# Ouranosinc/xclim

Hardware: AMD Instinct MI355X
Metric: grid-cells x timesteps / s (tx90p = percentile_doy + threshold_count + missing mask) (higher is better)
Workload: dtype f32; 1 GPU; tx90p (percentile_doy window 5 per 90 + threshold_count > + MissingAny) on 365x1440x720 fp32 per GPU, noleap, freq YS, time-major, resident in HBM

## Files before the change

xclim_amd/csrc/quantile.hip:

```cpp
#include <stdlib.h>

#include <type_traits>

#include "pdoy.h"

template <typename Getter>
__device__ __forceinline__ double xh_hf_quantile(int L, int n, double q, double alpha, double beta, Getter get) {
  if (L == 1) return (double)get(0);
  if (n < 2) {
    return n == 1 ? (double)get(0) : xh_nan64();
  }
  double nn = (double)n;
  double vi = nn * q + (alpha + q * (1.0 - alpha - beta)) - 1.0;
  if (vi >= nn - 1.0) return (double)get(n - 1);
  if (vi < 0.0) {
    const float v0 = get(0);
    return (v0 - v0 != 0.0f) ? (double)get(n - 1) : (double)v0;
  }
  double prev = floor(vi);
  int ip = (int)prev;
  double gamma = vi - prev;
  float left = get(ip), right = get(ip + 1);
  float diff = right - left;
  double r = (double)left + (double)diff * gamma;
// ... 47 lines not shown
      int64_t t = tb - half + k;
      okm[i] = inb && tb >= 0 && t >= 0 && t < T;
      raw[i] = xh_load<VEC>(x + (okm[i] ? t : (int64_t)0) * st + c);
    }
#pragma unroll
    for (int i = 0; i < NMAX; ++i) {
#pragma unroll
      for (int v = 0; v < VEC; ++v) {
        const uint32_t kk = okm[i] ? xh_f2key(raw[i].v[v]) : 0xFFFFFFFFu;
        key[v][i] = kk;
        nvalid[v] += (kk != 0xFFFFFFFFu) ? 1 : 0;
      }
    }
#pragma unroll
    for (int v = 0; v < VEC; ++v) {
      bitonic_regs<NMAX>(key[v]);
      auto get = [&](int idx) -> float {
        uint32_t r = 0;
#pragma unroll
        for (int i = 0; i < NMAX; ++i) r |= (i == idx) ? key[v][i] : 0u;
        return xh_key2f(r);
      };
      for (int j = 0; j < nper; ++j) {
        double r = xh_hf_quantile(N, nvalid[v], qs[j], alpha, beta, get);
        out[((int64_t)j * ndoy + d) * C + c + v] = r;
      }
    }
  }
}

__device__ __forceinline__ void ce(uint32_t& a, uint32_t& b) {
  uint32_t lo = a < b ? a : b, hi = a < b ? b : a;
  a = lo;
  b = hi;
}

template <int W>
__device__ __forceinline__ void sort_small(uint32_t (&k)[W]) {
  if (W == 1) return;
  if (W == 2) { ce(k[0], k[1 % W]); return; }
  if (W == 3) { ce(k[0], k[1 % W]); ce(k[1 % W], k[2 % W]); ce(k[0], k[1 % W]); return; }
  if (W == 5) {
    ce(k[0], k[1 % W]); ce(k[3 % W], k[4 % W]); ce(k[2 % W], k[4 % W]); ce(k[2 % W], k[3 % W]); ce(k[0], k[3 % W]);
    ce(k[0], k[2 % W]); ce(k[1 % W], k[4 % W]); ce(k[1 % W], k[3 % W]); ce(k[1 % W], k[2 % W]);
    return;
  }
#pragma unroll
  for (int r = 0; r < W; ++r) {
#pragma unroll
    for (int i = (r & 1); i + 1 < W; i += 2) ce(k[i], k[i + 1]);
  }
}

template <int W, int VEC, bool COUNT = false>
__global__ void __launch_bounds__(XH_BLOCK)
k_pdoy_slide(const float* __restrict__ x, int64_t T, int64_t C, int64_t st, int64_t t_first, int ndoy, int chunk,
             const QTab* __restrict__ qtab, int nper, double* __restrict__ out, int fast, int op = 0,
             const int32_t* __restrict__ doy_period = nullptr, int32_t* __restrict__ cnt_out = nullptr,
             int32_t* __restrict__ valid_out = nullptr) {
  __shared__ QTab s_tab[8 * (W + 1)];
  for (int i = threadIdx.x; i < nper * (W + 1); i += XH_BLOCK) s_tab[i] = qtab[i];
  __syncthreads();
  constexpr int NP = VEC == 4 ? 2 : 1;
  constexpr int GW = VEC == 4 ? 2 : 1;
  const int lane = threadIdx.x & 63;
  const int64_t wbase = ((int64_t)blockIdx.x * XH_BLOCK + (threadIdx.x & ~63)) * VEC;
  if (wbase >= C) return;
  int64_t cg[NP];
  bool okg[NP];
#pragma unroll
  for (int g = 0; g < NP; ++g) {
    cg[g] = wbase + (VEC == 4 ? 2 * lane + 128 * g : lane);
    okg[g] = cg[g] < C;
  }
  auto cell = [&](int v) -> int64_t { return cg[v / GW] + v % GW; };
  constexpr int half = W / 2;
  int d0 = blockIdx.y * chunk, d1 = d0 + chunk;
  if (d1 > ndoy) d1 = ndoy;
  uint32_t win[VEC][W];
  int n[VEC];
#pragma unroll
  for (int v = 0; v < VEC; ++v) {
    n[v] = 0;
#pragma unroll
    for (int k = 0; k < W; ++k) win[v][k] = 0xFFFFFFFFu;
  }
  auto fetch = [&](int64_t t) -> VecF<VEC> {
    const int64_t tc = t < 0 ? 0 : (t >= T ? T - 1 : t);
    const float* row = x + tc * st;
    VecF<VEC> r;
#pragma unroll
    for (int g = 0; g < NP; ++g) {
      const VecF<GW> h = xh_load<GW>(row + (okg[g] ? cg[g] : C - GW));
#pragma unroll
      for (int k = 0; k < GW; ++k) r.v[(g * GW + k) % VEC] = h.v[k];
    }
    return r;
  };
  int ccnt[VEC], cval[VEC], cper = -1;
#pragma unroll
  for (int v = 0; v < VEC; ++v) { ccnt[v] = 0; cval[v] = 0; }
  auto flush_counts = [&]() {
    if (cper >= 0) {
#pragma unroll
      for (int v = 0; v < VEC; ++v) {
        if (ccnt[v] && okg[v / GW]) atomicAdd(&cnt_out[(int64_t)cper * C + cell(v)], ccnt[v]);
        if (valid_out && cval[v] && okg[v / GW]) atomicAdd(&valid_out[(int64_t)cper * C + cell(v)], cval[v]);
        ccnt[v] = 0; cval[v] = 0;
      }
    }
  };
  auto emit = [&](int d, int j, const double (&r)[VEC], const uint32_t (&centre)[VEC]) {
    if (COUNT) {
      const int p = doy_period[d];
// ... 459 lines not shown
  hipLaunchKernelGGL(k_pdoy_lds, grid, dim3(64), lds, ctx->stream, x, T, C, st, d_tbase, nyears, ndoy, window, NP, cw, d_q, nper,
                     alpha, beta, out, d_vmap, Tv, d_doy_list, ndl);
  XH_LAUNCH_CHECK();
  return XH_OK;
}

static int launch_pdoy(xh_ctx* ctx, const float* x, int64_t T, int64_t C, int64_t st, const int32_t* d_tbase, int nyears,
                       int ndoy, int window, const double* d_q, int nper, double alpha, double beta, double* out) {
  int N = nyears * window;
  unsigned gy = (unsigned)(ndoy > 1024 ? 1024 : ndoy);
  if (N <= 8 && xh_pick_vec(x, C, st) == 4) {
    dim3 grid((unsigned)cdiv64(cdiv64(C, 4), XH_BLOCK), gy);
    hipLaunchKernelGGL((k_pdoy_reg<8, 4>), grid, dim3(XH_BLOCK), 0, ctx->stream, x, T, C, st, d_tbase, nyears, ndoy,
                       window, d_q, nper, alpha, beta, out);
  } else if (N <= 8) {
    dim3 grid((unsigned)cdiv64(C, XH_BLOCK), gy);
    hipLaunchKernelGGL((k_pdoy_reg<8, 1>), grid, dim3(XH_BLOCK), 0, ctx->stream, x, T, C, st, d_tbase, nyears, ndoy,
                       window, d_q, nper, alpha, beta, out);
  } else if (N <= 16) {
    dim3 grid((unsigned)cdiv64(C, XH_BLOCK), gy);
    hipLaunchKernelGGL((k_pdoy_reg<16, 1>), grid, dim3(XH_BLOCK), 0, ctx->stream, x, T, C, st, d_tbase, nyears, ndoy,
                       window, d_q, nper, alpha, beta, out);
  } else if (N <= 32) {
    dim3 grid((unsigned)cdiv64(C, XH_BLOCK), gy);
    hipLaunchKernelGGL((k_pdoy_reg<32, 1>), grid, dim3(XH_BLOCK), 0, ctx->stream, x, T, C, st, d_tbase, nyears, ndoy,
                       window, d_q, nper, alpha, beta, out);
  } else {
    return launch_pdoy_lds(ctx, x, T, C, st, d_tbase, nyears, ndoy, window, d_q, nper, alpha, beta, out, nullptr, T, nullptr,
                           0);
  }
  XH_LAUNCH_CHECK();
  return XH_OK;
}

static int slide_fast_mode(const QTab* tab, int nper, int W) {
  bool allmax = W > 1, allmin = W > 1;
  for (int j = 0; j < nper; ++j) {
    const QTab& e = tab[j * (W + 1) + W];
    allmax = allmax && e.lo == e.hi && e.lo == W - 1;
    allmin = allmin && e.lo == e.hi && e.lo == 0;
  }
  return allmax ? 1 : (allmin ? 2 : 0);
}

static int pdoy_impl(xh_ctx* ctx, const float* x, int64_t T, int64_t C, int64_t st, const int32_t* tbase, int nyears,
                     int ndoy, int window, const double* qh, int nper, double alpha, double beta, const int32_t* vmap,
                     int64_t Tv, double* out) {
  size_t cur = 0;
  void *d_tb = nullptr, *d_q = nullptr, *d_vmap = nullptr;
  const int N = nyears * window;
  bool contiguous = !vmap && nyears == 1 && nper <= 8 && (window == 3 || window == 5 || window == 7) && tbase[0] >= 0;
  for (int d = 1; contiguous && d < ndoy; ++d) contiguous = tbase[d] == tbase[0] + d;
  if (contiguous) {
    QTab tab[8 * 8];
    build_qtab(window, qh, nper, alpha, beta, tab);
    void* d_tab = nullptr;
    int rc = xh_scratch_upload(ctx, &cur, tab, sizeof(QTab) * (size_t)nper * (window + 1), &d_tab);
    if (rc) return rc;
    int chunk = 32;
    if (const char* e = xh_diag_env("XH_PDOY_SLIDE_CHUNK")) chunk = atoi(e) > 0 ? atoi(e) : chunk;
    const int vec = slide_vec(x, C, st, out);
    dim3 grid((unsigned)cdiv64(cdiv64(C, vec), XH_BLOCK), (unsigned)((ndoy + chunk - 1) / chunk));
#define XH_SLIDE(W, V)                                                                                              \
  hipLaunchKernelGGL((k_pdoy_slide<W, V>), grid, dim3(XH_BLOCK), 0, ctx->stream, x, T, C, st, (int64_t)tbase[0], ndoy, \
                     chunk, (const QTab*)d_tab, nper, out, slide_fast_mode(tab, nper, window))
    if (vec == 4) {
      if (window == 3) XH_SLIDE(3, 4); else if (window == 5) XH_SLIDE(5, 4); else XH_SLIDE(7, 4);
    } else {
      if (window == 3) XH_SLIDE(3, 1); else if (window == 5) XH_SLIDE(5, 1); else XH_SLIDE(7, 1);
    }
#undef XH_SLIDE
    XH_LAUNCH_CHECK();
    return XH_OK;
  }
  int rc = xh_scratch_upload(ctx, &cur, tbase, sizeof(int32_t) * (size_t)nyears * ndoy, &d_tb);
  if (rc) return rc;
  rc = xh_scratch_upload(ctx, &cur, qh, sizeof(double) * nper, &d_q);
  if (rc) return rc;
  if (vmap) {
    rc = xh_scratch_upload(ctx, &cur, vmap, sizeof(int32_t) * (size_t)Tv, &d_vmap);
    if (rc) return rc;
  }
  if (!vmap && N <= 32)
    return launch_pdoy(ctx, x, T, C, st, (const int32_t*)d_tb, nyears, ndoy, window, (const double*)d_q, nper, alpha, beta,
                       out);
  const bool mergeable = N > 32 && nyears <= 64 && (window == 3 || window == 5 || window == 7) && nper <= 16;
  if (!mergeable)
    return launch_pdoy_lds(ctx, x, T, C, st, (const int32_t*)d_tb, nyears, ndoy, window, (const double*)d_q, nper, alpha,
                           beta, out, (const int32_t*)d_vmap, Tv, nullptr, 0);
  uint8_t* regular = (uint8_t*)malloc((size_t)ndoy);
  int32_t* irregular = (int32_t*)malloc(sizeof(int32_t) * (size_t)ndoy);
  QTab* tab = (QTab*)malloc(sizeof(QTab) * (size_t)nper * (N + 1));
  if (!regular || !irregular || !tab) {
    free(regular); free(irregular); free(tab);
    xh_set_error("xh_percentile_doy: out of host memory");
    return XH_ERR_ARG;
  }
  const int nirr = pdoy_regular_flags(tbase, nyears, ndoy, window, T, vmap, Tv, regular, irregular);
  build_qtab(N, qh, nper, alpha, beta, tab);
  int32_t jtop[64], jbot[64], jrest[64];
  int ntop = 0, nbot = 0, nrest = 0;
  for (int j = 0; j < nper; ++j) {
    int dt = 0, db = 0;
    for (int n = 0; n <= N; ++n) {
      const QTab& e = tab[j * (N + 1) + n];
      if (e.lo < 0) continue;
      if (n - e.lo > dt) dt = n - e.lo;
      if (e.hi + 1 > db) db = e.hi + 1;
    }
    if (dt <= 16) jtop[ntop++] = j;
    else if (db <= 16) jbot[nbot++] = j;
    else jrest[nrest++] = j;
  }
  auto ring_depth = [&](const int32_t* js, int nj, int* pKT, int* pKB) {
    int kt = 1, kb = 0;
    for (int jj = 0; jj < nj; ++jj)
      for (int n = 0; n <= N; ++n) {
        const QTab& e = tab[js[jj] * (N + 1) + n];
// ... 36 lines not shown
  if (nbot) {
    rc = xh_launch_pdoy_top16(ctx, x, T, C, st, (const int32_t*)d_tb, nyears, ndoy, window, (const QTab*)d_tab,
                              (const int32_t*)d_jbot, nbot, 1, out, (const int32_t*)d_vmap, Tv, (const uint8_t*)d_reg);
    if (rc) return rc;
  }
  if (nrest == 0 && nirr == 0) return XH_OK;
  if (nrest) {
    const int rw = xh_launch_pdoy_walk(ctx, x, T, C, st, (const int32_t*)d_tb, nyears, ndoy, window, (const QTab*)d_tab,
                                       (const int32_t*)d_jrest, nrest, out, (const int32_t*)d_vmap, Tv, (const uint8_t*)d_reg);
    if (rw == XH_OK) nrest = 0;
    else if (rw != XH_ERR_NOTIMPL) return rw;
    if (nrest == 0 && nirr == 0) return XH_OK;
  }
  const size_t lds = ((size_t)window * (KT + KB) * 64 + (size_t)window * 64) * sizeof(uint32_t);
  const size_t lds_a = ((size_t)window * (KTa + KBa) * 64 + (size_t)window * 64) * sizeof(uint32_t);
#define XH_MERGE(W, NY)                                                                                                    \
  do {                                                                                                                     \
    if (nrest) {                                                                                                           \
      if (lds > 64 * 1024)                                                                                                 \
        XH_CHECK_HIP(hipFuncSetAttribute((const void*)k_pdoy_merge<W, NY, false>,                                          \
                                         hipFuncAttributeMaxDynamicSharedMemorySize, (int)lds));                           \
      hipLaunchKernelGGL((k_pdoy_merge<W, NY, false>), grid, dim3(64), lds, ctx->stream, x, T, C, st, (const int32_t*)d_tb, \
                         nyears, ndoy, chunk, (const QTab*)d_tab, (const int32_t*)d_jrest, nrest, out,                      \
                         (const int32_t*)d_vmap, Tv, (const uint8_t*)d_reg, (const int32_t*)nullptr, 0, KT, KB, abl);       \
    }                                                                                                                      \
    if (nirr) {                                                                                                            \
      if (lds_a > 64 * 1024)                                                                                               \
        XH_CHECK_HIP(hipFuncSetAttribute((const void*)k_pdoy_merge<W, NY, true>,                                           \
                                         hipFuncAttributeMaxDynamicSharedMemorySize, (int)lds_a));                         \
      hipLaunchKernelGGL((k_pdoy_merge<W, NY, true>), grid_irr, dim3(64), lds_a, ctx->stream, x, T, C, st,                  \
                         (const int32_t*)d_tb, nyears, ndoy, chunk, (const QTab*)d_tab, (const int32_t*)d_jall, nper, out,  \
                         (const int32_t*)d_vmap, Tv, (const uint8_t*)d_reg, (const int32_t*)d_irr, nirr, KTa, KBa, abl);    \
    }                                                                                                                      \
  } while (0)
  if (NYP == 32) {
    if (window == 3) XH_MERGE(3, 32); else if (window == 5) XH_MERGE(5, 32); else XH_MERGE(7, 32);
  } else {
    if (window == 3) XH_MERGE(3, 64); else if (window == 5) XH_MERGE(5, 64); else XH_MERGE(7, 64);
  }
#undef XH_MERGE
  XH_LAUNCH_CHECK();
  return XH_OK;
}

static int pdoy_count_impl(xh_ctx* ctx, const float* x, int64_t T, int64_t C, int64_t st, const int32_t* tbase, int ndoy,
                           int window, double per, double alpha, double beta, int op, const int32_t* doy_period, int P,
                           int32_t* count_out, int32_t* valid_out) {
  bool contiguous = (window == 3 || window == 5 || window == 7) && tbase[0] >= 0;
  for (int d = 1; contiguous && d < ndoy; ++d) contiguous = tbase[d] == tbase[0] + d;
  if (!contiguous) return XH_ERR_NOTIMPL;
  for (int d = 0; d < ndoy; ++d)
    XH_REQUIRE(doy_period[d] >= 0 && doy_period[d] < P, XH_ERR_ARG, "xh_percentile_doy_count: doy_period[%d] outside [0, P)", d);
  size_t cur = 0;
  QTab tab[8];
  const double q = per / 100.0;
  build_qtab(window, &q, 1, alpha, beta, tab);
  void *d_tab = nullptr, *d_dp = nullptr;
  int rc = xh_scratch_upload(ctx, &cur, tab, sizeof(QTab) * (size_t)(window + 1), &d_tab);
  if (!rc) rc = xh_scratch_upload(ctx, &cur, doy_period, sizeof(int32_t) * (size_t)ndoy, &d_dp);
  if (rc) return rc;
  XH_CHECK_HIP(hipMemsetAsync(count_out, 0, sizeof(int32_t) * (size_t)P * (size_t)C, ctx->stream));
  if (valid_out) XH_CHECK_HIP(hipMemsetAsync(valid_out, 0, sizeof(int32_t) * (size_t)P * (size_t)C, ctx->stream));
  int chunk = 61;
  if (const char* e = xh_diag_env("XH_PDOY_SLIDE_COUNT_CHUNK")) chunk = atoi(e) > 0 ? atoi(e) : chunk;
  const int vec = slide_vec(x, C, st, nullptr);
  dim3 grid((unsigned)cdiv64(cdiv64(C, vec), XH_BLOCK), (unsigned)((ndoy + chunk - 1) / chunk));
#define XH_SLIDEC(W, V)                                                                                                   \
  hipLaunchKernelGGL((k_pdoy_slide<W, V, true>), grid, dim3(XH_BLOCK), 0, ctx->stream, x, T, C, st, (int64_t)tbase[0], ndoy, \
                     chunk, (const QTab*)d_tab, 1, (double*)nullptr, slide_fast_mode(tab, 1, window), op,          \
                     (const int32_t*)d_dp, count_out, valid_out)
  if (vec == 4) {
    if (window == 3) XH_SLIDEC(3, 4); else if (window == 5) XH_SLIDEC(5, 4); else XH_SLIDEC(7, 4);
  } else {
    if (window == 3) XH_SLIDEC(3, 1); else if (window == 5) XH_SLIDEC(5, 1); else XH_SLIDEC(7, 1);
  }
#undef XH_SLIDEC
  XH_LAUNCH_CHECK();
  return XH_OK;
}

static int pdoy_count_multi(xh_ctx* ctx, const float* x, int64_t T, int64_t C, int64_t st, const int32_t* tbase, int nyears,
                            int ndoy, int window, double per, double alpha, double beta, int op, const int32_t* doy_period,
                            int P, int32_t* count_out, int32_t* valid_out) {
  const int N = nyears * window;
  if (!(N > 32 && nyears <= 64 && (window == 3 || window == 5 || window == 7))) return XH_ERR_NOTIMPL;
  if (op != XH_OP_GT && op != XH_OP_GE && op != XH_OP_LT && op != XH_OP_LE) return XH_ERR_NOTIMPL;
  for (int64_t i = 0; i < (int64_t)nyears * ndoy; ++i) {
    XH_REQUIRE(tbase[i] >= -1 && tbase[i] < T, XH_ERR_ARG, "xh_percentile_doy_count: tbase entry out of range");
    XH_REQUIRE(tbase[i] < 0 ? doy_period[i] < 0 : (doy_period[i] >= 0 && doy_period[i] < P), XH_ERR_ARG,
               "xh_percentile_doy_count: doy_period[%lld] must be in [0, P) for present days and < 0 for absent ones",
               (long long)i);
  }
  uint8_t* regular = (uint8_t*)malloc((size_t)ndoy);
  int32_t* irregular = (int32_t*)malloc(sizeof(int32_t) * (size_t)ndoy);
  QTab* tab = (QTab*)malloc(sizeof(QTab) * (size_t)(N + 1));
  if (!regular || !irregular || !tab) {
    free(regular); free(irregular); free(tab);
    xh_set_error("xh_percentile_doy_count: out of host memory");
    return XH_ERR_ARG;
  }
  const int nirr = pdoy_regular_flags(tbase, nyears, ndoy, window, T, nullptr, T, regular, irregular);
  const double q = per / 100.0;
  build_qtab(N, &q, 1, alpha, beta, tab);
  int dt = 0, db = 0;
  for (int n = 0; n <= N; ++n) {
    const QTab& e = tab[n];
    if (e.lo < 0) continue;
    if (n - e.lo > dt) dt = n - e.lo;
    if (e.hi + 1 > db) db = e.hi + 1;
  }
  const bool top = dt <= 16, bot = !top && db <= 16;
  const bool table_ok = nirr == 0 && (top || bot);
  int rc = table_ok ? XH_OK : XH_ERR_NOTIMPL;
  uint8_t* newseg = (uint8_t*)malloc((size_t)ndoy);
  if (!newseg) rc = XH_ERR_ARG;
  for (int d = 0; !rc && d < ndoy; ++d) {
    int nchg = 0, npres = 0;
    for (int y = 0; y < nyears; ++y) {
      const int32_t p1 = doy_period[(int64_t)y * ndoy + d], p0 = d > 0 ? doy_period[(int64_t)y * ndoy + d - 1] : p1;
      if (p1 < 0 || p0 < 0) continue;
      npres++;
      nchg += p1 != p0 ? 1 : 0;
// ... 168 lines not shown
```

xclim_amd/csrc/reduce.hip:

```cpp
#include "common.h"
#include "window.h"

template <int VEC, int KIND>
__global__ void __launch_bounds__(XH_BLOCK)
k_threshold_count(const float* __restrict__ x, int64_t C, int64_t st, int op, float thr32, double thr64,
                  const void* __restrict__ table, int64_t tstride, const int32_t* __restrict__ tidx,
                  const int64_t* __restrict__ seg_off, int P, int32_t* __restrict__ count_out,
                  int32_t* __restrict__ valid_out, int period_fast) {
  const unsigned tile = period_fast ? blockIdx.y : blockIdx.x;
  const int pstart = period_fast ? blockIdx.x : blockIdx.y, pstep = period_fast ? gridDim.x : gridDim.y;
  int64_t c = ((int64_t)tile * XH_BLOCK + threadIdx.x) * VEC;
  if (c >= C) return;
  for (int p = pstart; p < P; p += pstep) {
    int64_t t0 = seg_off[p], t1 = seg_off[p + 1];
    int cnt[VEC], val[VEC];
#pragma unroll
    for (int i = 0; i < VEC; ++i) cnt[i] = 0, val[i] = 0;
    xh_march_rows<VEC, 8>(x + c, st, t0, t1, [&](int64_t t, const VecF<VEC>& xv) {
      if (KIND == XH_THR_SCALAR_F32) {
#pragma unroll
        for (int i = 0; i < VEC; ++i) cnt[i] += xh_cmp_f32(xv.v[i], op, thr32) ? 1 : 0;
      } else if (KIND == XH_THR_SCALAR_F64) {
#pragma unroll
        for (int i = 0; i < VEC; ++i) cnt[i] += xh_cmp_f64((double)xv.v[i], op, thr64) ? 1 : 0;
// ... 7 lines not shown
          th[0] = a.x; th[1 % VEC] = a.y; th[2 % VEC] = b.x; th[3 % VEC] = b.y;
        } else {
#pragma unroll
          for (int i = 0; i < VEC; ++i) th[i] = tp[i];
        }
#pragma unroll
        for (int i = 0; i < VEC; ++i) cnt[i] += xh_cmp_f64((double)xv.v[i], op, th[i]) ? 1 : 0;
      } else {
        int64_t row = (KIND == XH_THR_DOY_F32) ? (int64_t)tidx[t] : t;
        VecF<VEC> th = xh_load<VEC>(reinterpret_cast<const float*>(table) + row * tstride + c);
#pragma unroll
        for (int i = 0; i < VEC; ++i) cnt[i] += xh_cmp_f32(xv.v[i], op, th.v[i]) ? 1 : 0;
      }
#pragma unroll
      for (int i = 0; i < VEC; ++i) val[i] += (xv.v[i] == xv.v[i]) ? 1 : 0;
    });
    int64_t o = (int64_t)p * C + c;
#pragma unroll
    for (int i = 0; i < VEC; ++i) count_out[o + i] = cnt[i];
    if (valid_out) {
#pragma unroll
      for (int i = 0; i < VEC; ++i) valid_out[o + i] = val[i];
    }
  }
}

template <int VEC>
static int launch_threshold_count(xh_ctx* ctx, int kind, dim3 grid, const float* x, int64_t C, int64_t st, int op,
                                  double thr, const void* table, int64_t tstride, const int32_t* tidx,
                                  const int64_t* seg, int P, int32_t* count_out, int32_t* valid_out, int period_fast) {
#define XH_TC(K)                                                                                                      \
  case K:                                                                                                             \
    hipLaunchKernelGGL((k_threshold_count<VEC, K>), grid, dim3(XH_BLOCK), 0, ctx->stream, x, C, st, op, (float)thr, thr, \
                       table, tstride, tidx, seg, P, count_out, valid_out, period_fast);                              \
    break;
  switch (kind) {
    XH_TC(XH_THR_SCALAR_F32)
    XH_TC(XH_THR_SCALAR_F64)
    XH_TC(XH_THR_DOY_F64)
    XH_TC(XH_THR_DOY_F32)
    XH_TC(XH_THR_FULL_F64)
    XH_TC(XH_THR_FULL_F32)
    default:
      xh_set_error("xh_threshold_count: unknown thr_kind %d", kind);
      return XH_ERR_ARG;
  }
#undef XH_TC
  XH_LAUNCH_CHECK();
  return XH_OK;
}

static inline unsigned period_grid(int P) { return (unsigned)(P < 1 ? 1 : (P > 4096 ? 4096 : P)); }

template <int VEC, bool FAST = false>
__global__ void __launch_bounds__(XH_BLOCK)
k_domain_count(const float* __restrict__ x, int64_t C, int64_t st, int op1, float thr1, int op2, float thr2, int combine,
               const int64_t* __restrict__ seg_off, int P, int32_t* __restrict__ count_out,
               int32_t* __restrict__ valid_out) {
  int64_t c = ((int64_t)blockIdx.x * XH_BLOCK + threadIdx.x) * VEC;
  if (c >= C) return;
  for (int p = blockIdx.y; p < P; p += gridDim.y) {
    int64_t t0 = seg_off[p], t1 = seg_off[p + 1];
    int cnt[VEC], val[VEC];
#pragma unroll
    for (int i = 0; i < VEC; ++i) cnt[i] = 0, val[i] = 0;
    xh_march_rows<VEC, 8>(x + c, st, t0, t1, [&](int64_t, const VecF<VEC>& xv) {
#pragma unroll
      for (int i = 0; i < VEC; ++i) {
        bool a, b;
        if (FAST) {
          a = xv.v[i] * __int_as_float(op1) > thr1;
          b = xv.v[i] * __int_as_float(op2) > thr2;
        } else {
          a = xh_cmp_f32(xv.v[i], op1, thr1);
          b = xh_cmp_f32(xv.v[i], op2, thr2);
        }
        cnt[i] += ((combine == 1) ? (a && b) : (a || b)) ? 1 : 0;
        val[i] += (xv.v[i] == xv.v[i]) ? 1 : 0;
      }
    });
    int64_t o = (int64_t)p * C + c;
#pragma unroll
    for (int i = 0; i < VEC; ++i) count_out[o + i] = cnt[i];
    if (valid_out) {
#pragma unroll
      for (int i = 0; i < VEC; ++i) valid_out[o + i] = val[i];
    }
  }
}

template <int VEC, int RED>
__global__ void __launch_bounds__(XH_BLOCK)
k_resample_reduce(const float* __restrict__ x, int64_t C, int64_t st, int skipna, const int64_t* __restrict__ seg_off,
                  int P, void* __restrict__ out_v, int32_t* __restrict__ valid_out) {
  int64_t c = ((int64_t)blockIdx.x * XH_BLOCK + threadIdx.x) * VEC;
  if (c >= C) return;
  for (int p = blockIdx.y; p < P; p += gridDim.y) {
    int64_t t0 = seg_off[p], t1 = seg_off[p + 1];
    double s1[VEC], s2[VEC];
    float ext[VEC];
    int n[VEC], arg[VEC], nanseen[VEC];
#pragma unroll
    for (int i = 0; i < VEC; ++i) {
      s1[i] = 0.0; s2[i] = 0.0; n[i] = 0; arg[i] = -1; nanseen[i] = 0;
      ext[i] = 0.f;
    }
// ... 37 lines not shown
            if (!nanseen[i] && !skipna && (RED == XH_RED_ARGMIN || RED == XH_RED_ARGMAX)) arg[i] = (int)(t - t0);
            nanseen[i] = 1;
          }
        }
      });
    }
    int64_t o = (int64_t)p * C + c;
    int len = (int)(t1 - t0);
#pragma unroll
    for (int i = 0; i < VEC; ++i) {
      bool poisoned = (!skipna && nanseen[i]);
      if (RED == XH_RED_COUNT) {
        reinterpret_cast<int32_t*>(out_v)[o + i] = n[i];
      } else if (RED == XH_RED_ARGMIN || RED == XH_RED_ARGMAX) {
        reinterpret_cast<int32_t*>(out_v)[o + i] = arg[i];
      } else {
        float r;
        if (RED == XH_RED_SUM) r = poisoned ? xh_nan32() : (float)s1[i];
        else if (RED == XH_RED_MEAN) r = (poisoned || n[i] == 0) ? xh_nan32() : (float)(s1[i] / (double)n[i]);
        else if (RED == XH_RED_MIN || RED == XH_RED_MAX) r = (poisoned || n[i] == 0) ? xh_nan32() : ext[i];
        else if (RED == XH_RED_VAR) r = (poisoned || n[i] == 0) ? xh_nan32() : (float)(s2[i] / (double)n[i]);
        else r = (poisoned || n[i] == 0) ? xh_nan32() : (float)sqrt(s2[i] / (double)n[i]);
        if (len == 0 && RED != XH_RED_SUM) r = xh_nan32();
        reinterpret_cast<float*>(out_v)[o + i] = r;
      }
    }
    if (valid_out) {
#pragma unroll
      for (int i = 0; i < VEC; ++i) valid_out[o + i] = n[i];
    }
  }
}

template <int VEC>
static int launch_resample_reduce(xh_ctx* ctx, int reducer, dim3 grid, const float* x, int64_t C, int64_t st, int skipna,
                                  const int64_t* seg, int P, void* out, int32_t* valid_out) {
#define XH_RR(R)                                                                                                   \
  case R:                                                                                                          \
    hipLaunchKernelGGL((k_resample_reduce<VEC, R>), grid, dim3(XH_BLOCK), 0, ctx->stream, x, C, st, skipna, seg, P, out, \
                       valid_out);                                                                                 \
    break;
  switch (reducer) {
    XH_RR(XH_RED_SUM) XH_RR(XH_RED_MEAN) XH_RR(XH_RED_MIN) XH_RR(XH_RED_MAX) XH_RR(XH_RED_STD) XH_RR(XH_RED_VAR)
    XH_RR(XH_RED_COUNT) XH_RR(XH_RED_ARGMIN) XH_RR(XH_RED_ARGMAX)
    default:
      xh_set_error("xh_resample_reduce: reducer %d not recognized", reducer);
      return XH_ERR_OP;
  }
#undef XH_RR
  XH_LAUNCH_CHECK();
  return XH_OK;
}

__global__ void __launch_bounds__(XH_BLOCK)
k_apply_missing_mask(const void* __restrict__ value, int kind, const int32_t* __restrict__ valid,
                     const int32_t* __restrict__ expected, int P, int64_t C, double* __restrict__ out) {
  int64_t i = (int64_t)blockIdx.x * XH_BLOCK + threadIdx.x;
  int64_t n = (int64_t)P * C;
  if (i >= n) return;
  int p = (int)(i / C);
  double v = kind == 0 ? (double)reinterpret_cast<const int32_t*>(value)[i]
             : kind == 1 ? (double)reinterpret_cast<const float*>(value)[i]
                         : reinterpret_cast<const double*>(value)[i];
  out[i] = (valid[i] != expected[p]) ? xh_nan64() : v;
}

template <int RED>
__global__ void __launch_bounds__(XH_BLOCK)
k_rolling_reduce(const float* __restrict__ x, int64_t T, int64_t C, int64_t st, int window, int left, int right,
                 float* __restrict__ out, int64_t out_st) {
  int64_t c = (int64_t)blockIdx.x * XH_BLOCK + threadIdx.x;
  if (c >= C) return;
  int64_t chunk = cdiv64(T, (int64_t)gridDim.y);
  int64_t ta = (int64_t)blockIdx.y * chunk, tb = ta + chunk;
  if (tb > T) tb = T;
  for (int64_t t = ta; t < tb; ++t) {
    int64_t a = t - left, b = t + right;
    float r;
    if (RED == XH_RED_COUNT) {
      int n = 0;
      for (int64_t k = (a < 0 ? 0 : a); k <= b && k < T; ++k) {
        float v = x[k * st + c];
        n += (v == v) ? 1 : 0;
      }
      r = (float)n;
    } else if (a < 0 || b >= T) {
      r = xh_nan32();
    } else {
      double s = 0.0;
      float e = x[a * st + c];
      bool nan = false;
      for (int64_t k = a; k <= b; ++k) {
        float v = x[k * st + c];
        nan |= (v != v);
        if (RED == XH_RED_MIN) e = v < e ? v : e;
        else if (RED == XH_RED_MAX) e = v > e ? v : e;
        else s += (double)v;
      }
      if (RED == XH_RED_SUM) r = (float)s;
      else if (RED == XH_RED_MEAN) r = (float)(s / (double)window);
      else if (RED == XH_RED_MIN || RED == XH_RED_MAX) r = e;
      else {
        double m = s / (double)window, s2 = 0.0;
        for (int64_t k = a; k <= b; ++k) {
          double d = (double)x[k * st + c] - m;
          s2 += d * d;
        }
        r = (RED == XH_RED_VAR) ? (float)(s2 / (double)window) : (float)sqrt(s2 / (double)window);
      }
      if (nan) r = xh_nan32();
    }
    out[t * out_st + c] = r;
  }
}

static int check_tc(const char* fn, xh_ctx* ctx, const void* x, int64_t T, int64_t C, int64_t st, int64_t sc) {
  XH_REQUIRE(ctx && x, XH_ERR_ARG, "%s: NULL argument", fn);
  XH_REQUIRE(T >= 0 && C >= 0, XH_ERR_ARG, "%s: negative shape", fn);
  XH_REQUIRE(sc == 1 && st >= C, XH_ERR_LAYOUT,
             "%s: streaming kernels need a time-major view (sc == 1, st >= C); got st=%lld sc=%lld — transpose first",
             fn, (long long)st, (long long)sc);
  return XH_OK;
}

static int upload_segments(xh_ctx* ctx, size_t* cur, const int64_t* seg_off, int P, int64_t T, const char* fn,
                           const int64_t** d_seg) {
  XH_REQUIRE(seg_off && P >= 1, XH_ERR_ARG, "%s: seg_off NULL or P < 1", fn);
  for (int p = 0; p < P; ++p)
    XH_REQUIRE(seg_off[p] <= seg_off[p + 1] && seg_off[p] >= 0 && seg_off[p + 1] <= T, XH_ERR_ARG,
               "%s: seg_off must be non-decreasing within [0, T]", fn);
  void* d = nullptr;
  int rc = xh_scratch_upload(ctx, cur, seg_off, sizeof(int64_t) * (size_t)(P + 1), &d);
  if (rc) return rc;
  *d_seg = (const int64_t*)d;
  return XH_OK;
}

extern "C" {

static int threshold_count_impl(xh_ctx* ctx, const float* x, int64_t T, int64_t C, int64_t st, int64_t sc, int op, int thr_kind,
                                double thr_scalar, const void* thr_table, int64_t thr_stride, const int32_t* tidx,
                                const int64_t* seg_off, int P, int32_t* count_out, int32_t* valid_out, int ndoy) {
  int rc = check_tc("xh_threshold_count", ctx, x, T, C, st, sc);
  if (rc) return rc;
  XH_REQUIRE(op >= XH_OP_GT && op <= XH_OP_NE, XH_ERR_OP, "Operation `%d` not recognized.", op);
  XH_REQUIRE(count_out, XH_ERR_ARG, "xh_threshold_count: count_out is NULL");
  if (thr_kind >= XH_THR_DOY_F64) {
    XH_REQUIRE(thr_table && thr_stride >= C, XH_ERR_ARG, "xh_threshold_count: threshold table missing or stride < C");
    if (thr_kind == XH_THR_DOY_F64 || thr_kind == XH_THR_DOY_F32)
      XH_REQUIRE(tidx, XH_ERR_ARG, "xh_threshold_count: tidx required for per-doy thresholds");
  }
  size_t cur = 0;
  const int64_t* d_seg = nullptr;
  rc = upload_segments(ctx, &cur, seg_off, P, T, "xh_threshold_count", &d_seg);
  if (rc) return rc;
  if (C == 0) return XH_OK;
  if (thr_kind == XH_THR_DOY_F64 && ndoy > 0 && !xh_diag_env("XH_TCOUNT_LEGACY")) {
    rc = xh_launch_tcount_doy(ctx, x, T, C, st, op, static_cast<const double*>(thr_table), thr_stride, tidx, d_seg, seg_off, P,
                              ndoy, count_out, valid_out);
    if (rc != XH_ERR_NOTIMPL) return rc;
  }
  int vec = xh_pick_vec(x, C, st);
  if (thr_kind >= XH_THR_DOY_F64) {
    size_t esz = (thr_kind == XH_THR_DOY_F64 || thr_kind == XH_THR_FULL_F64) ? 8 : 4;
    if ((reinterpret_cast<uintptr_t>(thr_table) & 15) != 0 || (thr_stride * esz) % 16 != 0) vec = 1;
  }
  unsigned tiles = (unsigned)cdiv64(cdiv64(C, vec), XH_BLOCK);
  const bool doy = thr_kind == XH_THR_DOY_F64 || thr_kind == XH_THR_DOY_F32;
  const int period_fast = (doy && P > 1 && tiles <= 65535u) ? 1 : 0;
  dim3 grid = period_fast ? dim3(period_grid(P), tiles) : dim3(tiles, period_grid(P));
  if (vec == 4)
    return launch_threshold_count<4>(ctx, thr_kind, grid, x, C, st, op, thr_scalar, thr_table, thr_stride, tidx, d_seg, P,
                                     count_out, valid_out, period_fast);
  return launch_threshold_count<1>(ctx, thr_kind, grid, x, C, st, op, thr_scalar, thr_table, thr_stride, tidx, d_seg, P,
                                   count_out, valid_out, period_fast);
}

int xh_threshold_count(xh_ctx* ctx, const float* x, int64_t T, int64_t C, int64_t st, int64_t sc, int op, int thr_kind,
                       double thr_scalar, const void* thr_table, int64_t thr_stride, const int32_t* tidx,
                       const int64_t* seg_off, int P, int32_t* count_out, int32_t* valid_out) {
  return threshold_count_impl(ctx, x, T, C, st, sc, op, thr_kind, thr_scalar, thr_table, thr_stride, tidx, seg_off, P, count_out,
                              valid_out, 0);
}

int xh_threshold_count_doy(xh_ctx* ctx, const float* x, int64_t T, int64_t C, int64_t st, int64_t sc, int op,
                           const double* thr_table, int64_t thr_stride, int ndoy, const int32_t* tidx, const int64_t* seg_off,
                           int P, int32_t* count_out, int32_t* valid_out) {
  XH_REQUIRE(ndoy >= 1, XH_ERR_ARG, "xh_threshold_count_doy: the table needs at least one row (ndoy = %d)", ndoy);
  return threshold_count_impl(ctx, x, T, C, st, sc, op, XH_THR_DOY_F64, 0.0, thr_table, thr_stride, tidx, seg_off, P, count_out,
                              valid_out, ndoy);
}

int xh_domain_count(xh_ctx* ctx, const float* x, int64_t T, int64_t C, int64_t st, int64_t sc, int op1, double thr1,
                    int op2, double thr2, int combine, const int64_t* seg_off, int P, int32_t* count_out,
                    int32_t* valid_out) {
  int rc = check_tc("xh_domain_count", ctx, x, T, C, st, sc);
  if (rc) return rc;
  XH_REQUIRE(op1 >= XH_OP_GT && op1 <= XH_OP_NE && op2 >= XH_OP_GT && op2 <= XH_OP_NE, XH_ERR_OP,
             "Operation `%d/%d` not recognized.", op1, op2);
  XH_REQUIRE(combine == 1 || combine == 2, XH_ERR_ARG, "xh_domain_count: combine must be 1 (and) or 2 (or)");
  XH_REQUIRE(count_out, XH_ERR_ARG, "xh_domain_count: count_out is NULL");
  size_t cur = 0;
  const int64_t* d_seg = nullptr;
  rc = upload_segments(ctx, &cur, seg_off, P, T, "xh_domain_count", &d_seg);
  if (rc) return rc;
  if (C == 0) return XH_OK;
  int vec = xh_pick_vec(x, C, st);
  dim3 grid((unsigned)cdiv64(cdiv64(C, vec), XH_BLOCK), period_grid(P));
  const XhOneCmp c1 = xh_one_cmp(op1, (float)thr1), c2 = xh_one_cmp(op2, (float)thr2);
  if (vec == 4 && c1.ok && c2.ok) {
    int s1, s2;
    memcpy(&s1, &c1.sgn, 4);
    memcpy(&s2, &c2.sgn, 4);
    hipLaunchKernelGGL((k_domain_count<4, true>), grid, dim3(XH_BLOCK), 0, ctx->stream, x, C, st, s1, c1.thr, s2, c2.thr, combine,
                       d_seg, P, count_out, valid_out);
  } else if (vec == 4)
    hipLaunchKernelGGL((k_domain_count<4>), grid, dim3(XH_BLOCK), 0, ctx->stream, x, C, st, op1, (float)thr1, op2,
                       (float)thr2, combine, d_seg, P, count_out, valid_out);
  else
    hipLaunchKernelGGL((k_domain_count<1>), grid, dim3(XH_BLOCK), 0, ctx->stream, x, C, st, op1, (float)thr1, op2,
                       (float)thr2, combine, d_seg, P, count_out, valid_out);
  XH_LAUNCH_CHECK();
  return XH_OK;
}

int xh_resample_reduce(xh_ctx* ctx, const float* x, int64_t T, int64_t C, int64_t st, int64_t sc, int reducer, int skipna,
                       const int64_t* seg_off, int P, void* out, int32_t* valid_out) {
  int rc = check_tc("xh_resample_reduce", ctx, x, T, C, st, sc);
  if (rc) return rc;
  XH_REQUIRE(out, XH_ERR_ARG, "xh_resample_reduce: out is NULL");
  size_t cur = 0;
  const int64_t* d_seg = nullptr;
  rc = upload_segments(ctx, &cur, seg_off, P, T, "xh_resample_reduce", &d_seg);
  if (rc) return rc;
  if (C == 0) return XH_OK;
  int vec = xh_pick_vec(x, C, st);
  dim3 grid((unsigned)cdiv64(cdiv64(C, vec), XH_BLOCK), period_grid(P));
  if (vec == 4) return launch_resample_reduce<4>(ctx, reducer, grid, x, C, st, skipna, d_seg, P, out, valid_out);
  return launch_resample_reduce<1>(ctx, reducer, grid, x, C, st, skipna, d_seg, P, out, valid_out);
}

int xh_apply_missing_mask(xh_ctx* ctx, const void* value, int value_kind, const int32_t* valid, const int32_t* expected,
                          int P, int64_t C, double* out64) {
  XH_REQUIRE(ctx && value && valid && expected && out64, XH_ERR_ARG, "xh_apply_missing_mask: NULL argument");
  XH_REQUIRE(value_kind >= 0 && value_kind <= 2, XH_ERR_ARG, "xh_apply_missing_mask: value_kind must be 0, 1 or 2");
  XH_REQUIRE(P >= 1 && C >= 0, XH_ERR_ARG, "xh_apply_missing_mask: bad shape");
  size_t cur = 0;
  void* d_exp = nullptr;
  int rc = xh_scratch_upload(ctx, &cur, expected, sizeof(int32_t) * (size_t)P, &d_exp);
  if (rc) return rc;
  int64_t n = (int64_t)P * C;
  if (n == 0) return XH_OK;
  hipLaunchKernelGGL(k_apply_missing_mask, dim3((unsigned)cdiv64(n, XH_BLOCK)), dim3(XH_BLOCK), 0, ctx->stream, value,
                     value_kind, valid, (const int32_t*)d_exp, P, C, out64);
  XH_LAUNCH_CHECK();
  return XH_OK;
}

int xh_rolling_reduce(xh_ctx* ctx, const float* x, int64_t T, int64_t C, int64_t st, int64_t sc, int window, int center,
                      int reducer, float* out, int64_t out_st) {
  int rc = check_tc("xh_rolling_reduce", ctx, x, T, C, st, sc);
  if (rc) return rc;
  XH_REQUIRE(out && out_st >= C, XH_ERR_ARG, "xh_rolling_reduce: out NULL or out_st < C");
  XH_REQUIRE(window >= 1, XH_ERR_ARG, "xh_rolling_reduce: window must be >= 1");
  if (T == 0 || C == 0) return XH_OK;
  int left = center ? window / 2 : window - 1;
  int right = window - 1 - left;
  {
    int rr = xh_launch_rolling_ring(ctx, x, T, C, st, window, left, right, reducer, out, out_st);
    if (rr != XH_ERR_NOTIMPL) return rr;
  }
  unsigned ny = (unsigned)(T < 64 ? T : 64);
  dim3 grid((unsigned)cdiv64(C, XH_BLOCK), ny);
#define XH_RO(R)                                                                                                      \
  case R:                                                                                                             \
    hipLaunchKernelGGL((k_rolling_reduce<R>), grid, dim3(XH_BLOCK), 0, ctx->stream, x, T, C, st, window, left, right, out, \
                       out_st);                                                                                       \
    break;
  switch (reducer) {
    XH_RO(XH_RED_SUM) XH_RO(XH_RED_MEAN) XH_RO(XH_RED_MIN) XH_RO(XH_RED_MAX) XH_RO(XH_RED_STD) XH_RO(XH_RED_VAR)
    XH_RO(XH_RED_COUNT)
    default:
      xh_set_error("xh_rolling_reduce: reducer %d not recognized", reducer);
      return XH_ERR_OP;
  }
#undef XH_RO
  XH_LAUNCH_CHECK();
  return XH_OK;
}

}
```

Baseline: 231.9 billion cell-timesteps/s.

## Pass small tables as kernel args and add year-wise threshold count kernel

Quantile tables, segment offsets and expected counts are now passed by value in kernel arguments instead of being uploaded to device scratch memory, which removes host-to-device copies before each launch. A new k_tcount_year kernel counts per-doy threshold exceedances with 4-wide vector loads, nontemporal loads, a 4-step time unroll with prefetched tidx, and a fixed waves-per-EU hint. It is used when the planned LDS path is unavailable or declined. Larger kernel argument blocks and a new code path add risk, and the occupancy hint may not suit every shape.

```diff
diff --git a/xclim_amd/csrc/quantile.hip b/xclim_amd/csrc/quantile.hip
--- a/xclim_amd/csrc/quantile.hip
+++ b/xclim_amd/csrc/quantile.hip
@@ -123,14 +123,17 @@
   }
 }
 
+struct QTabArg {
+  QTab e[8 * 8];
+};
 template <int W, int VEC, bool COUNT = false>
 __global__ void __launch_bounds__(XH_BLOCK)
 k_pdoy_slide(const float* __restrict__ x, int64_t T, int64_t C, int64_t st, int64_t t_first, int ndoy, int chunk,
-             const QTab* __restrict__ qtab, int nper, double* __restrict__ out, int fast, int op = 0,
+             const QTabArg qtab, int nper, double* __restrict__ out, int fast, int op = 0,
              const int32_t* __restrict__ doy_period = nullptr, int32_t* __restrict__ cnt_out = nullptr,
              int32_t* __restrict__ valid_out = nullptr) {
   __shared__ QTab s_tab[8 * (W + 1)];
-  for (int i = threadIdx.x; i < nper * (W + 1); i += XH_BLOCK) s_tab[i] = qtab[i];
+  for (int i = threadIdx.x; i < nper * (W + 1); i += XH_BLOCK) s_tab[i] = qtab.e[i];
   __syncthreads();
   constexpr int NP = VEC == 4 ? 2 : 1;
   constexpr int GW = VEC == 4 ? 2 : 1;
@@ -696,18 +699,17 @@
   bool contiguous = !vmap && nyears == 1 && nper <= 8 && (window == 3 || window == 5 || window == 7) && tbase[0] >= 0;
   for (int d = 1; contiguous && d < ndoy; ++d) contiguous = tbase[d] == tbase[0] + d;
   if (contiguous) {
-    QTab tab[8 * 8];
+    QTabArg targ;
+    memset(&targ, 0, sizeof(targ));
+    QTab* tab = targ.e;
     build_qtab(window, qh, nper, alpha, beta, tab);
-    void* d_tab = nullptr;
-    int rc = xh_scratch_upload(ctx, &cur, tab, sizeof(QTab) * (size_t)nper * (window + 1), &d_tab);
-    if (rc) return rc;
     int chunk = 32;
     if (const char* e = xh_diag_env("XH_PDOY_SLIDE_CHUNK")) chunk = atoi(e) > 0 ? atoi(e) : chunk;
     const int vec = slide_vec(x, C, st, out);
     dim3 grid((unsigned)cdiv64(cdiv64(C, vec), XH_BLOCK), (unsigned)((ndoy + chunk - 1) / chunk));
 #define XH_SLIDE(W, V)                                                                                              \
   hipLaunchKernelGGL((k_pdoy_slide<W, V>), grid, dim3(XH_BLOCK), 0, ctx->stream, x, T, C, st, (int64_t)tbase[0], ndoy, \
-                     chunk, (const QTab*)d_tab, nper, out, slide_fast_mode(tab, nper, window))
+                     chunk, targ, nper, out, slide_fast_mode(tab, nper, window))
     if (vec == 4) {
       if (window == 3) XH_SLIDE(3, 4); else if (window == 5) XH_SLIDE(5, 4); else XH_SLIDE(7, 4);
     } else {
@@ -850,12 +852,13 @@
   for (int d = 0; d < ndoy; ++d)
     XH_REQUIRE(doy_period[d] >= 0 && doy_period[d] < P, XH_ERR_ARG, "xh_percentile_doy_count: doy_period[%d] outside [0, P)", d);
   size_t cur = 0;
-  QTab tab[8];
+  QTabArg targ;
+  memset(&targ, 0, sizeof(targ));
+  QTab* tab = targ.e;
   const double q = per / 100.0;
   build_qtab(window, &q, 1, alpha, beta, tab);
-  void *d_tab = nullptr, *d_dp = nullptr;
-  int rc = xh_scratch_upload(ctx, &cur, tab, sizeof(QTab) * (size_t)(window + 1), &d_tab);
-  if (!rc) rc = xh_scratch_upload(ctx, &cur, doy_period, sizeof(int32_t) * (size_t)ndoy, &d_dp);
+  void* d_dp = nullptr;
+  int rc = xh_scratch_upload(ctx, &cur, doy_period, sizeof(int32_t) * (size_t)ndoy, &d_dp);
   if (rc) return rc;
   XH_CHECK_HIP(hipMemsetAsync(count_out, 0, sizeof(int32_t) * (size_t)P * (size_t)C, ctx->stream));
   if (valid_out) XH_CHECK_HIP(hipMemsetAsync(valid_out, 0, sizeof(int32_t) * (size_t)P * (size_t)C, ctx->stream));
@@ -865,7 +868,7 @@
   dim3 grid((unsigned)cdiv64(cdiv64(C, vec), XH_BLOCK), (unsigned)((ndoy + chunk - 1) / chunk));
 #define XH_SLIDEC(W, V)                                                                                                   \
   hipLaunchKernelGGL((k_pdoy_slide<W, V, true>), grid, dim3(XH_BLOCK), 0, ctx->stream, x, T, C, st, (int64_t)tbase[0], ndoy, \
-                     chunk, (const QTab*)d_tab, 1, (double*)nullptr, slide_fast_mode(tab, 1, window), op,          \
+                     chunk, targ, 1, (double*)nullptr, slide_fast_mode(tab, 1, window), op,                        \
                      (const int32_t*)d_dp, count_out, valid_out)
   if (vec == 4) {
     if (window == 3) XH_SLIDEC(3, 4); else if (window == 5) XH_SLIDEC(5, 4); else XH_SLIDEC(7, 4);
diff --git a/xclim_amd/csrc/reduce.hip b/xclim_amd/csrc/reduce.hip
--- a/xclim_amd/csrc/reduce.hip
+++ b/xclim_amd/csrc/reduce.hip
@@ -83,6 +83,100 @@
 
 static inline unsigned period_grid(int P) { return (unsigned)(P < 1 ? 1 : (P > 4096 ? 4096 : P)); }
 
+#define XH_TCY_R 4
+#define XH_SEG_ARG_MAX 32
+struct XhSegArg {
+  int64_t off[XH_SEG_ARG_MAX + 1];
+};
+#if defined(__HIP_DEVICE_COMPILE__)
+#define XH_TCY_WAVES __attribute__((amdgpu_waves_per_eu(4, 4)))
+#else
+#define XH_TCY_WAVES
+#endif
+
+#if defined(__clang__)
+typedef float tcy_f4 __attribute__((ext_vector_type(4)));
+typedef double tcy_d2 __attribute__((ext_vector_type(2)));
+__device__ __forceinline__ float4 tcy_load(const float* p) {
+  const tcy_f4 t = __builtin_nontemporal_load(reinterpret_cast<const tcy_f4*>(p));
+  return make_float4(t.x, t.y, t.z, t.w);
+}
+__device__ __forceinline__ double2 tcy_load(const double* p) {
+  const tcy_d2 t = __builtin_nontemporal_load(reinterpret_cast<const tcy_d2*>(p));
+  return make_double2(t.x, t.y);
+}
+#else
+__device__ __forceinline__ float4 tcy_load(const float* p) { return *reinterpret_cast<const float4*>(p); }
+__device__ __forceinline__ double2 tcy_load(const double* p) { return *reinterpret_cast<const double2*>(p); }
+#endif
+
+template <int OP, bool SEGARG>
+__global__ void __launch_bounds__(XH_BLOCK) XH_TCY_WAVES
+k_tcount_year(const float* __restrict__ x, int64_t C, int64_t st, const double* __restrict__ table, int64_t tstride,
+              const int32_t* __restrict__ tidx, const int64_t* __restrict__ seg_ptr, const XhSegArg seg_val, int P,
+              int32_t* __restrict__ count_out, int32_t* __restrict__ valid_out, int period_fast) {
+  constexpr int R = XH_TCY_R;
+  const unsigned tile = period_fast ? blockIdx.y : blockIdx.x;
+  const int pstart = period_fast ? blockIdx.x : blockIdx.y, pstep = period_fast ? gridDim.x : gridDim.y;
+  const int64_t c = ((int64_t)tile * XH_BLOCK + threadIdx.x) * 4;
+  if (c >= C) return;
+  const float* __restrict__ xc = x + c;
+  const double* __restrict__ tc = table + c;
+  for (int p = pstart; p < P; p += pstep) {
+    const int64_t t0 = SEGARG ? seg_val.off[p] : seg_ptr[p], t1 = SEGARG ? seg_val.off[p + 1] : seg_ptr[p + 1];
+    int cnt[4] = {0, 0, 0, 0}, val[4] = {0, 0, 0, 0};
+    auto tally = [&](const float4& v, const double2& a, const double2& b) {
+      cnt[0] += xh_cmp_f64((double)v.x, OP, a.x) ? 1 : 0;
+      cnt[1] += xh_cmp_f64((double)v.y, OP, a.y) ? 1 : 0;
+      cnt[2] += xh_cmp_f64((double)v.z, OP, b.x) ? 1 : 0;
+      cnt[3] += xh_cmp_f64((double)v.w, OP, b.y) ? 1 : 0;
+      val[0] += (v.x == v.x) ? 1 : 0;
+      val[1] += (v.y == v.y) ? 1 : 0;
+      val[2] += (v.z == v.z) ? 1 : 0;
+      val[3] += (v.w == v.w) ? 1 : 0;
+    };
+    const int64_t nfull = (t1 - t0) / R;
+    int64_t tb = t0;
+    int32_t nxt[R] = {};
+    if (nfull > 0) {
+#pragma unroll
+      for (int r = 0; r < R; ++r) nxt[r] = tidx[tb + r];
+    }
+    for (int64_t k = 0; k < nfull; ++k) {
+      int64_t row[R];
+#pragma unroll
+      for (int r = 0; r < R; ++r) row[r] = (int64_t)nxt[r];
+      const int64_t tn = k + 1 < nfull ? tb + R : tb;
+#pragma unroll
+      for (int r = 0; r < R; ++r) nxt[r] = tidx[tn + r];
+      float4 v[R];
+      double2 a[R], b[R];
+#pragma unroll
+      for (int r = 0; r < R; ++r) {
+        v[r] = tcy_load(xc + (tb + r) * st);
+        const double* tp = tc + row[r] * tstride;
+        a[r] = tcy_load(tp);
+        b[r] = tcy_load(tp + 2);
+      }
+#pragma unroll
+      for (int r = 0; r < R; ++r) tally(v[r], a[r], b[r]);
+      tb = tn;
+    }
+    for (int64_t t = t0 + nfull * R; t < t1; ++t) {
+      const float4 v = tcy_load(xc + t * st);
+      const double* tp = tc + (int64_t)tidx[t] * tstride;
+      tally(v, tcy_load(tp), tcy_load(tp + 2));
+    }
+    const int64_t o = (int64_t)p * C + c;
+#pragma unroll
+    for (int i = 0; i < 4; ++i) count_out[o + i] = cnt[i];
+    if (valid_out) {
+#pragma unroll
+      for (int i = 0; i < 4; ++i) valid_out[o + i] = val[i];
+    }
+  }
+}
+
 template <int VEC, bool FAST = false>
 __global__ void __launch_bounds__(XH_BLOCK)
 k_domain_count(const float* __restrict__ x, int64_t C, int64_t st, int op1, float thr1, int op2, float thr2, int combine,
@@ -226,9 +320,15 @@
   return XH_OK;
 }
 
+#define XH_EXP_ARG_MAX 64
+struct XhExpArg {
+  int32_t n[XH_EXP_ARG_MAX];
+};
+
 __global__ void __launch_bounds__(XH_BLOCK)
 k_apply_missing_mask(const void* __restrict__ value, int kind, const int32_t* __restrict__ valid,
-                     const int32_t* __restrict__ expected, int P, int64_t C, double* __restrict__ out) {
+                     const int32_t* __restrict__ expected, const XhExpArg exp_val, int P, int64_t C,
+                     double* __restrict__ out) {
   int64_t i = (int64_t)blockIdx.x * XH_BLOCK + threadIdx.x;
   int64_t n = (int64_t)P * C;
   if (i >= n) return;
@@ -236,7 +336,7 @@
   double v = kind == 0 ? (double)reinterpret_cast<const int32_t*>(value)[i]
              : kind == 1 ? (double)reinterpret_cast<const float*>(value)[i]
                          : reinterpret_cast<const double*>(value)[i];
-  out[i] = (valid[i] != expected[p]) ? xh_nan64() : v;
+  out[i] = (valid[i] != (expected ? expected[p] : exp_val.n[p])) ? xh_nan64() : v;
 }
 
 template <int RED>
@@ -297,16 +397,44 @@
   return XH_OK;
 }
 
-static int upload_segments(xh_ctx* ctx, size_t* cur, const int64_t* seg_off, int P, int64_t T, const char* fn,
-                           const int64_t** d_seg) {
+static int check_segments(const int64_t* seg_off, int P, int64_t T, const char* fn) {
   XH_REQUIRE(seg_off && P >= 1, XH_ERR_ARG, "%s: seg_off NULL or P < 1", fn);
   for (int p = 0; p < P; ++p)
     XH_REQUIRE(seg_off[p] <= seg_off[p + 1] && seg_off[p] >= 0 && seg_off[p + 1] <= T, XH_ERR_ARG,
                "%s: seg_off must be non-decreasing within [0, T]", fn);
+  return XH_OK;
+}
+
+static int upload_segments(xh_ctx* ctx, size_t* cur, const int64_t* seg_off, int P, int64_t T, const char* fn,
+                           const int64_t** d_seg) {
+  int rc = check_segments(seg_off, P, T, fn);
+  if (rc) return rc;
   void* d = nullptr;
-  int rc = xh_scratch_upload(ctx, cur, seg_off, sizeof(int64_t) * (size_t)(P + 1), &d);
+  rc = xh_scratch_upload(ctx, cur, seg_off, sizeof(int64_t) * (size_t)(P + 1), &d);
   if (rc) return rc;
   *d_seg = (const int64_t*)d;
+  return XH_OK;
+}
+
+static int launch_tcount_year(xh_ctx* ctx, dim3 grid, const float* x, int64_t C, int64_t st, int op, const double* table,
+                              int64_t tstride, const int32_t* tidx, const int64_t* d_seg, const int64_t* h_seg, int P,
+                              int32_t* count_out, int32_t* valid_out, int period_fast) {
+  XhSegArg sv;
+  memset(&sv, 0, sizeof(sv));
+  if (!d_seg) memcpy(sv.off, h_seg, sizeof(int64_t) * (size_t)(P + 1));
+#define XH_TCY2(OPV, BYVAL)                                                                                              \
+  hipLaunchKernelGGL((k_tcount_year<OPV, BYVAL>), grid, dim3(XH_BLOCK), 0, ctx->stream, x, C, st, table, tstride, tidx, d_seg, \
+                     sv, P, count_out, valid_out, period_fast)
+#define XH_TCY(OPV)                                  \
+  case OPV:                                          \
+    if (d_seg) XH_TCY2(OPV, false); else XH_TCY2(OPV, true); \
+    break;
+  switch (op) {
+    XH_TCY(XH_OP_GT) XH_TCY(XH_OP_LT) XH_TCY(XH_OP_GE) XH_TCY(XH_OP_LE) XH_TCY(XH_OP_EQ) XH_TCY(XH_OP_NE)
+  }
+#undef XH_TCY
+#undef XH_TCY2
+  XH_LAUNCH_CHECK();
   return XH_OK;
 }
 
@@ -324,25 +452,42 @@
     if (thr_kind == XH_THR_DOY_F64 || thr_kind == XH_THR_DOY_F32)
       XH_REQUIRE(tidx, XH_ERR_ARG, "xh_threshold_count: tidx required for per-doy thresholds");
   }
+  rc = check_segments(seg_off, P, T, "xh_threshold_count");
+  if (rc) return rc;
   size_t cur = 0;
   const int64_t* d_seg = nullptr;
-  rc = upload_segments(ctx, &cur, seg_off, P, T, "xh_threshold_count", &d_seg);
-  if (rc) return rc;
-  if (C == 0) return XH_OK;
-  if (thr_kind == XH_THR_DOY_F64 && ndoy > 0 && !xh_diag_env("XH_TCOUNT_LEGACY")) {
-    rc = xh_launch_tcount_doy(ctx, x, T, C, st, op, static_cast<const double*>(thr_table), thr_stride, tidx, d_seg, seg_off, P,
-                              ndoy, count_out, valid_out);
-    if (rc != XH_ERR_NOTIMPL) return rc;
+  const bool legacy = xh_diag_env("XH_TCOUNT_LEGACY") != nullptr;
+  if (thr_kind == XH_THR_DOY_F64 && ndoy > 0 && !legacy && C > 0) {
+    int64_t longest = 0;
+    for (int p = 0; p < P; ++p) longest = seg_off[p + 1] - seg_off[p] > longest ? seg_off[p + 1] - seg_off[p] : longest;
+    size_t lds = 0;
+    int narrow = 0;
+    if (xh_tcount_plan(T, C, st, op, P, ndoy, longest, &lds, &narrow) == XH_OK) {
+      rc = upload_segments(ctx, &cur, seg_off, P, T, "xh_threshold_count", &d_seg);
+      if (rc) return rc;
+      rc = xh_launch_tcount_doy(ctx, x, T, C, st, op, static_cast<const double*>(thr_table), thr_stride, tidx, d_seg, seg_off, P,
+                                ndoy, count_out, valid_out);
+      if (rc != XH_ERR_NOTIMPL) return rc;
+    }
   }
   int vec = xh_pick_vec(x, C, st);
   if (thr_kind >= XH_THR_DOY_F64) {
     size_t esz = (thr_kind == XH_THR_DOY_F64 || thr_kind == XH_THR_FULL_F64) ? 8 : 4;
     if ((reinterpret_cast<uintptr_t>(thr_table) & 15) != 0 || (thr_stride * esz) % 16 != 0) vec = 1;
   }
+  const bool year = thr_kind == XH_THR_DOY_F64 && vec == 4 && !legacy && !xh_diag_env("XH_TCOUNT_ROWWISE");
+  if (!d_seg && !(year && P <= XH_SEG_ARG_MAX)) {
+    rc = upload_segments(ctx, &cur, seg_off, P, T, "xh_threshold_count", &d_seg);
+    if (rc) return rc;
+  }
+  if (C == 0) return XH_OK;
   unsigned tiles = (unsigned)cdiv64(cdiv64(C, vec), XH_BLOCK);
   const bool doy = thr_kind == XH_THR_DOY_F64 || thr_kind == XH_THR_DOY_F32;
   const int period_fast = (doy && P > 1 && tiles <= 65535u) ? 1 : 0;
   dim3 grid = period_fast ? dim3(period_grid(P), tiles) : dim3(tiles, period_grid(P));
+  if (year)
+    return launch_tcount_year(ctx, grid, x, C, st, op, static_cast<const double*>(thr_table), thr_stride, tidx, d_seg, seg_off, P,
+                              count_out, valid_out, period_fast);
   if (vec == 4)
     return launch_threshold_count<4>(ctx, thr_kind, grid, x, C, st, op, thr_scalar, thr_table, thr_stride, tidx, d_seg, P,
                                      count_out, valid_out, period_fast);
@@ -421,12 +566,18 @@
   XH_REQUIRE(P >= 1 && C >= 0, XH_ERR_ARG, "xh_apply_missing_mask: bad shape");
   size_t cur = 0;
   void* d_exp = nullptr;
-  int rc = xh_scratch_upload(ctx, &cur, expected, sizeof(int32_t) * (size_t)P, &d_exp);
-  if (rc) return rc;
+  XhExpArg ev;
+  memset(&ev, 0, sizeof(ev));
+  if (P <= XH_EXP_ARG_MAX) {
+    memcpy(ev.n, expected, sizeof(int32_t) * (size_t)P);
+  } else {
+    int rc = xh_scratch_upload(ctx, &cur, expected, sizeof(int32_t) * (size_t)P, &d_exp);
+    if (rc) return rc;
+  }
   int64_t n = (int64_t)P * C;
   if (n == 0) return XH_OK;
   hipLaunchKernelGGL(k_apply_missing_mask, dim3((unsigned)cdiv64(n, XH_BLOCK)), dim3(XH_BLOCK), 0, ctx->stream, value,
-                     value_kind, valid, (const int32_t*)d_exp, P, C, out64);
+                     value_kind, valid, (const int32_t*)d_exp, ev, P, C, out64);
   XH_LAUNCH_CHECK();
   return XH_OK;
 }
```

New measurement: 240.9 billion cell-timesteps/s, median of 6. +3.9%, better.
